# meta-pytorch/torchx

Hardware: AMD Instinct MI355X
Metric: tokens_per_second (higher is better)
Workload: dtype bf16; 1 GPU; model=llama3_8b, global_batch=4, seq_len=4096, parallelism=dp1

## Files before the change

torchx_amd/ops/csrc/attention.hip:

```cpp
#include "common.h"

#include <cstdlib>
#include <cstring>
#include <type_traits>

typedef __bf16 mbf16x8 __attribute__((ext_vector_type(8)));

#define HD 128
#define QBLK 32
#define KBLK 32
#define NWAVES 4
#define BLOCK_Q (QBLK * NWAVES)
#define BLOCK_K (KBLK * NWAVES)

__device__ __forceinline__ f32x16 mfma32(mbf16x8 a, mbf16x8 b, f32x16 c) {
  return __builtin_amdgcn_mfma_f32_32x32x16_bf16(a, b, c, 0, 0, 0);
}

__device__ __forceinline__ unsigned int pack_bf16x2(float a, float b) {
  unsigned int r;
  asm("v_cvt_pk_bf16_f32 %0, %1, %2" : "=v"(r) : "v"(a), "v"(b));
  return r;
}

__device__ __forceinline__ int c_row(int r, int half) {
  return (r & 3) + 8 * (r >> 2) + 4 * half;
}

__device__ __forceinline__ void cvals_to_frags(const float* p, bool hi,
                                               mbf16x8* f0, mbf16x8* f1) {
  unsigned int w[2][4];
  #pragma unroll
  for (int s = 0; s < 2; ++s) {
    unsigned int a01 = pack_bf16x2(p[8 * s + 0], p[8 * s + 1]);
    unsigned int a23 = pack_bf16x2(p[8 * s + 2], p[8 * s + 3]);
    unsigned int a45 = pack_bf16x2(p[8 * s + 4], p[8 * s + 5]);
    unsigned int a67 = pack_bf16x2(p[8 * s + 6], p[8 * s + 7]);
    unsigned int x01 = __shfl_xor((int)a01, 32, 64);
    unsigned int x23 = __shfl_xor((int)a23, 32, 64);
    unsigned int x45 = __shfl_xor((int)a45, 32, 64);
    unsigned int x67 = __shfl_xor((int)a67, 32, 64);
    w[s][0] = hi ? x45 : a01;
    w[s][1] = hi ? x67 : a23;
    w[s][2] = hi ? a45 : x01;
    w[s][3] = hi ? a67 : x23;
  }
  uint4_v u0 = {w[0][0], w[0][1], w[0][2], w[0][3]};
  uint4_v u1 = {w[1][0], w[1][1], w[1][2], w[1][3]};
  *f0 = __builtin_bit_cast(mbf16x8, u0);
  *f1 = __builtin_bit_cast(mbf16x8, u1);
}


#define FKV 64
#define KIMG_BYTES (FKV * 256)
#define VIMG_BYTES (HD * FKV * 2)
#define LOG2E 1.44269504088896340736f
#define LN2 0.69314718055994530942f

__device__ __forceinline__ mbf16x8 kimg_frag(const char* kimg, int sub, int c) {
  const int lane = threadIdx.x & 63;
  const int row = sub * 32 + (lane & 31);
  const int byte = (c * 32 + ((lane >> 5) * 16)) ^ ((row & 15) << 4);
  return *(const mbf16x8*)(kimg + row * 256 + byte);
}

__device__ __forceinline__ int vrot(int d) {
  return ((d >> 1) ^ (d >> 4)) & 7;
}

__device__ __forceinline__ mbf16x8 vimg_frag(const char* vimg, int dt, int ks) {
  const int lane = threadIdx.x & 63;
  const int d = dt * 32 + (lane & 31);
  const int g = (ks * 2 + (lane >> 5) + vrot(d)) & 7;
  return *(const mbf16x8*)(vimg + d * 128 + g * 16);
}

typedef short short4_v __attribute__((ext_vector_type(4)));
typedef __attribute__((address_space(3))) short4_v* lds_s4p;

__device__ __forceinline__ mbf16x8 nat_tr_frag(const char* nat, int ks,
                                               int dt) {
  const int lane = threadIdx.x & 63;
  const int j = lane & 15;
  const int r_lo = ks * 16 + ((lane >> 5) * 8) + (j >> 2);
  const int r_hi = r_lo + 4;
  const int d0 = dt * 32 + ((lane >> 4) & 1) * 16 + 4 * (j & 3);
  const int g16 = (d0 >> 3) << 4;
  const int off = (d0 & 7) * 2;
  const int b_lo = r_lo * 256 + ((g16 ^ ((r_lo & 15) << 4)) | off);
  const int b_hi = r_hi * 256 + ((g16 ^ ((r_hi & 15) << 4)) | off);
  short4_v lo = __builtin_amdgcn_ds_read_tr16_b64_v4i16(
      (lds_s4p)(nat + b_lo));
  short4_v hi = __builtin_amdgcn_ds_read_tr16_b64_v4i16(
      (lds_s4p)(nat + b_hi));
  uint2_v ul = __builtin_bit_cast(uint2_v, lo);
  uint2_v uh = __builtin_bit_cast(uint2_v, hi);
  uint4_v u = {ul[0], ul[1], uh[0], uh[1]};
  return __builtin_bit_cast(mbf16x8, u);
}

template <int NW = 4, int TFKV = FKV>
__device__ __forceinline__ void stage_k_glds(
    const unsigned short* __restrict__ kb, long kv0, long stride_elems,
    int S, char* kimg) {
  const int wave = threadIdx.x / 64;
  const int lane = threadIdx.x & 63;
  #pragma unroll
  for (int j = 0; j < (TFKV / 4) / NW; ++j) {
    const int i = wave * ((TFKV / 4) / NW) + j;
    const int row = i * 4 + (lane >> 4);
    const int colbyte = ((lane & 15) * 16) ^ ((row & 15) << 4);
    long srow = kv0 + row;
    if (srow >= S) srow = S - 1;
    const char* src = (const char*)(kb + srow * stride_elems) + colbyte;
    __builtin_amdgcn_global_load_lds(
        (const __attribute__((address_space(1))) unsigned int*)src,
        (__attribute__((address_space(3))) unsigned int*)(kimg + i * 1024),
        16, 0, 0);
  }
}

__device__ __forceinline__ void load_v_regs(
    const unsigned short* __restrict__ vb, long kv0, long stride_elems,
    int S, ushort8 vr[4]) {
  const int tid = threadIdx.x;
  #pragma unroll
  for (int p = 0; p < 4; ++p) {
    const int c = tid + p * 256;
    const int r = c >> 4, g = c & 15;
    long srow = kv0 + r;
    if (srow >= S) srow = S - 1;
    vr[p] = *(const ushort8*)(vb + srow * stride_elems + g * 8);
  }
}

__device__ __forceinline__ void write_v_tr(const ushort8 vr[4], char* vimg) {
  const int tid = threadIdx.x;
  #pragma unroll
  for (int p = 0; p < 4; ++p) {
    const int c = tid + p * 256;
    const int r = c >> 4, g = c & 15;
    #pragma unroll
    for (int j = 0; j < 8; ++j) {
      const int d = 8 * g + j;
      const int gr = ((r >> 3) + vrot(d)) & 7;
      *(unsigned short*)(vimg + d * 128 + gr * 16 + (r & 7) * 2) = vr[p][j];
    }
  }
}


__device__ __forceinline__ void map_block_fwd(int B, int Hq, int Hkv,
                                              int nqt, int G,
                                              int* b, int* hq, int* qt) {
  int bid = blockIdx.x;
  if (((B * Hkv) & 7) == 0) {
    const int gsz = G * nqt;
    const int xcd = bid & 7, slot = bid >> 3;
    const int g = (slot / gsz) * 8 + xcd;
    *b = g / Hkv;
    const int r = slot % gsz;
    *hq = (g % Hkv) * G + r / nqt;
    *qt = r % nqt;
  } else {
    *b = bid / (Hq * nqt);
    bid -= *b * Hq * nqt;
    *hq = bid / nqt;
    *qt = bid % nqt;
  }
}

__device__ __forceinline__ bool map_block_fwd_balanced(int B, int Hq, int Hkv,
                                                       int nqt, int G,
                                                       int heavy, int* b,
                                                       int* hq, int* qt) {
  const int xcd = blockIdx.x & 7, slot = blockIdx.x >> 3;
  const int u = slot / G;
  const int nstream = B * Hkv;
  int g, t;
  if ((nstream & 7) == 0) {
    const int ns = nstream >> 3;
    g = (u % ns) * 8 + xcd;
    t = u / ns;
  } else {
    const int unit = u * 8 + xcd;
    if (unit >= nstream * nqt) return false;
    g = unit % nstream;
    t = unit / nstream;
  }
  *b = g / Hkv;
  *hq = (g % Hkv) * G + slot % G;
  *qt = heavy ? nqt - 1 - t : t;
  return true;
}

template <int NTHREADS>
__device__ __forceinline__ void lds_nat_to_tr(const char* nat, char* tr_img) {
  const int tid = threadIdx.x;
  #pragma unroll
  for (int p = 0; p < 1024 / NTHREADS; ++p) {
    const int c = tid + p * NTHREADS;
    const int r = c >> 4, g = c & 15;
    const ushort8 v = *(const ushort8*)(
        nat + r * 256 + ((g * 16) ^ ((r & 15) << 4)));
    #pragma unroll
    for (int j = 0; j < 8; ++j) {
      const int d = 8 * g + j;
      const int gr = ((r >> 3) + vrot(d)) & 7;
      *(unsigned short*)(tr_img + d * 128 + gr * 16 + (r & 7) * 2) = v[j];
    }
  }
}



template <int NW = 4>
__device__ __forceinline__ void lds_nat_to_tr_own(const char* nat,
                                                  char* tr_img) {
  const int wave = threadIdx.x / 64;
  const int lane = threadIdx.x & 63;
  #pragma unroll
  for (int pp = 0; pp < 16 / NW; ++pp) {
    const int c = wave * (64 * 16 / NW) + pp * 64 + lane;
    const int r = c >> 4, g = c & 15;
    const ushort8 v = *(const ushort8*)(
        nat + r * 256 + ((g * 16) ^ ((r & 15) << 4)));
    #pragma unroll
    for (int j = 0; j < 8; ++j) {
      const int d = 8 * g + j;
      const int gr = ((r >> 3) + vrot(d)) & 7;
      *(unsigned short*)(tr_img + d * 128 + gr * 16 + (r & 7) * 2) = v[j];
    }
  }
}

template <int NW>
__global__ void __launch_bounds__(NW * 64, 2)
attn_fwd_kernel(const unsigned short* __restrict__ q,
                const unsigned short* __restrict__ k,
                const unsigned short* __restrict__ v,
                unsigned short* __restrict__ o,
                float* __restrict__ lse,
                int B, int S, int Hq, int Hkv, float scale, int causal,
                long q_rs, long kv_rs,
                int map) {
  __shared__ __align__(16) char smem[4 * KIMG_BYTES];

  const int BQ = NW * QBLK;
  const int nqt = (S + BQ - 1) / BQ;
  const int G = Hq / Hkv;
  int b, hq, qt;
  if (map == 0) {
    map_block_fwd(B, Hq, Hkv, nqt, G, &b, &hq, &qt);
  } else if (!map_block_fwd_balanced(B, Hq, Hkv, nqt, G, map == 1, &b, &hq,
                                     &qt)) {
    return;
  }
  const int hkv = hq / G;

  const int wave = threadIdx.x / 64;
  const int lane = threadIdx.x & 63;
  const bool hi = lane >= 32;
  const int qr = lane & 31;

  const long q_seq_stride = q_rs;
  const long kv_seq_stride = kv_rs;
  const unsigned short* qb = q + (long)b * S * q_seq_stride + (long)hq * HD;
  const unsigned short* kb = k + (long)b * S * kv_seq_stride + (long)hkv * HD;
  const unsigned short* vb = v + (long)b * S * kv_seq_stride + (long)hkv * HD;

  const int q0_blk = qt * BQ;
  const int qw0 = q0_blk + wave * QBLK;
  const long q_row = qw0 + qr;
  const bool wave_active = qw0 < S;

  mbf16x8 qfrag[8];
  {
    const long row = (q_row < S) ? q_row : (S - 1);
    const unsigned short* qp = qb + row * q_seq_stride + (hi ? 8 : 0);
    #pragma unroll
    for (int c = 0; c < 8; ++c) {
      qfrag[c] = __builtin_bit_cast(mbf16x8, *(const ushort8*)(qp + c * 16));
    }
  }

  f32x16 acc_o[4] = {};
  float m_run = -3.0e38f, l_run = 0.f;
  const float sc2 = scale * LOG2E;

  const int kv_limit = causal ? min(S, q0_blk + BQ) : S;
  const int ntiles = (kv_limit + FKV - 1) / FKV;
  const int qw_max = min(qw0 + QBLK - 1, S - 1);

  char* k0 = smem;
  char* k1 = smem + KIMG_BYTES;
  char* vcur = smem + 2 * KIMG_BYTES;
  char* vnxt = smem + 3 * KIMG_BYTES;

  stage_k_glds<NW>(kb, 0, kv_seq_stride, S, k0);
  stage_k_glds<NW>(vb, 0, kv_seq_stride, S, vcur);
  asm volatile("s_waitcnt vmcnt(0)");
  __syncthreads();

  for (int t = 0; t < ntiles; ++t) {
    const int kv0 = t * FKV;
    const bool has_next = (t + 1) < ntiles;
    if (has_next) {
      stage_k_glds<NW>(kb, kv0 + FKV, kv_seq_stride, S, k1);
      stage_k_glds<NW>(vb, kv0 + FKV, kv_seq_stride, S, vnxt);
    }

    const bool needed = wave_active && (!causal || kv0 <= qw_max);
    if (needed) {
      f32x16 acc0 = {}, acc1 = {};
      __builtin_amdgcn_s_setprio(1);
      #pragma unroll
      for (int c = 0; c < 8; ++c) {
        acc0 = mfma32(kimg_frag(k0, 0, c), qfrag[c], acc0);
        acc1 = mfma32(kimg_frag(k0, 1, c), qfrag[c], acc1);
      }
      __builtin_amdgcn_s_setprio(0);

      float sv[32];
      #pragma unroll
      for (int r = 0; r < 16; ++r) {
        sv[r] = acc0[r] * sc2;
        sv[16 + r] = acc1[r] * sc2;
      }
      const bool mask_tile =
          (causal && kv0 + FKV - 1 > qw0) || (kv0 + FKV > S) || (q_row >= S);
      if (mask_tile) {
        #pragma unroll
        for (int r = 0; r < 32; ++r) {
          const long kg = kv0 + (r >> 4) * 32 + c_row(r & 15, hi);
          if (kg >= S || q_row >= S || (causal && kg > q_row)) {
            sv[r] = -3.0e38f;
          }
        }
      }

      float m_tile = sv[0];
      #pragma unroll
      for (int r = 1; r < 32; ++r) m_tile = fmaxf(m_tile, sv[r]);
      m_tile = fmaxf(m_tile, __shfl_xor(m_tile, 32, 64));
      const float THR2 = 11.54f;
      if (!__all(m_tile - m_run <= THR2)) {
        const float m_new = fmaxf(m_run, m_tile);
        const float alpha = __builtin_amdgcn_exp2f(m_run - m_new);
        l_run *= alpha;
        m_run = m_new;
        #pragma unroll
        for (int dt = 0; dt < 4; ++dt) {
          #pragma unroll
          for (int r = 0; r < 16; ++r) acc_o[dt][r] *= alpha;
        }
      }

      float row_sum = 0.f;
      #pragma unroll
      for (int r = 0; r < 32; ++r) {
        sv[r] = __builtin_amdgcn_exp2f(sv[r] - m_run);
        row_sum += sv[r];
      }
      row_sum += __shfl_xor(row_sum, 32, 64);
      l_run += row_sum;

      mbf16x8 pf[4];
      cvals_to_frags(sv, hi, &pf[0], &pf[1]);
      cvals_to_frags(sv + 16, hi, &pf[2], &pf[3]);

      __builtin_amdgcn_s_setprio(1);
      #pragma unroll
      for (int dt = 0; dt < 4; ++dt) {
        #pragma unroll
        for (int ks = 0; ks < 4; ++ks) {
          acc_o[dt] = mfma32(nat_tr_frag(vcur, ks, dt), pf[ks], acc_o[dt]);
        }
      }
      __builtin_amdgcn_s_setprio(0);
    }

    if (has_next) {
      asm volatile("s_waitcnt vmcnt(0)");
      __syncthreads();
      char* tk = k0; k0 = k1; k1 = tk;
      char* tv = vcur; vcur = vnxt; vnxt = tv;
    }
  }

  if (!wave_active || q_row >= S) return;

  const float inv_l = (l_run > 0.f) ? 1.0f / l_run : 0.f;
  unsigned short* ob =
      o + (((long)b * S + q_row) * Hq + hq) * HD;
  #pragma unroll
  for (int dt = 0; dt < 4; ++dt) {
    #pragma unroll
    for (int g = 0; g < 4; ++g) {
      bf16x4_raw w;
      #pragma unroll
      for (int j = 0; j < 4; ++j) {
        w[j] = (short)f32_to_bf16(acc_o[dt][4 * g + j] * inv_l);
      }
      *(bf16x4_raw*)(ob + dt * 32 + 8 * g + 4 * (hi ? 1 : 0)) = w;
    }
  }
  if (!hi) {
    lse[((long)b * Hq + hq) * S + q_row] = (m_run + __log2f(l_run)) * LN2;
  }
// ... 695 lines not shown
  const int nt = (S + TFKV - 1) / TFKV;
  const int nt_eff = nt - t0;
  const int total = G * nt_eff;

  const bool ds_on = is_dk && ds != nullptr;
  const int ds_nqt = (S + BLOCK_Q - 1) / BLOCK_Q;
  const long ds_plane = ds_qt_base(ds_nqt, ds_nqt, causal);
  const long ds_lane = (long)(kw0 / KBLK) * (4 * DS_IMG_BYTES) + kr * 64 +
                       (hi ? 16 : 0);

  auto head_q = [&](int gh) {
    return q + (long)b * S * q_seq_stride + (long)(hkv * G + gh) * HD;
  };
  auto head_do = [&](int gh) {
    return dout + (long)b * S * dout_rs + (long)(hkv * G + gh) * HD;
  };
  auto stage_lse = [&](int gh, int t, int buf) {
    const int hq_ = hkv * G + gh;
    const int q0_ = t * TFKV;
    if (threadIdx.x < TFKV) {
      const float* lse_b = lse + ((long)b * Hq + hq_) * S;
      const int qg = q0_ + threadIdx.x;
      lse_buf[buf][threadIdx.x] = (qg < S) ? lse_b[qg] * LOG2E : 0.f;
    } else if (threadIdx.x < 2 * TFKV) {
      const float* del_b = delta + ((long)b * Hq + hq_) * S;
      const int qg = q0_ + (threadIdx.x - TFKV);
      del_buf[buf][threadIdx.x - TFKV] = (qg < S) ? del_b[qg] : 0.f;
    }
  };

  stage_k_glds8<TFKV>(head_q(0), (long)t0 * TFKV, q_seq_stride, S, qn_c);
  stage_k_glds8<TFKV>(head_do(0), (long)t0 * TFKV, dout_rs, S, don_c);
  asm volatile("s_waitcnt vmcnt(0)");
  stage_lse(0, t0, 0);
  __syncthreads();

  const float* lse_cur = lse_buf[0];
  const float* del_cur = del_buf[0];
  int lse_nxt = 1;
  for (int idx = 0; idx < total; ++idx) {
    const int gh = idx / nt_eff;
    const int t = t0 + idx % nt_eff;
    const int q0 = t * TFKV;
    const int hq = hkv * G + gh;
    const bool has_next = (idx + 1) < total;
    const int ngh = (idx + 1) / nt_eff;
    const long nrow0 = (long)(t0 + (idx + 1) % nt_eff) * TFKV;
    if (has_next) {
      stage_k_glds8<TFKV>(head_q(ngh), nrow0, q_seq_stride, S, qn_n);
      stage_k_glds8<TFKV>(head_do(ngh), nrow0, dout_rs, S, don_n);
    }

    const bool needed =
        wave_active && (!causal || q0 + TFKV - 1 >= kw0);
    int n_ds = 0;
    if (needed) {
      char* ds_head = ds + ((long)b * Hq + hq) * ds_plane * (4 * DS_IMG_BYTES)
                      + ds_lane;
      #pragma clang loop unroll(disable)
      for (int sb = 0; sb < TFKV / 32; ++sb) {
        if (causal && q0 + 32 * sb + 32 <= kw0) continue;
        f32x16 acc_s = {}, acc_dp = {};
        #pragma unroll
        for (int c = 0; c < 8; ++c) {
          acc_s = mfma32(kimg_frag(qn_c, sb, c), kfrag[c], acc_s);
          if (is_dk) {
            acc_dp = mfma32(kimg_frag(don_c, sb, c), vfrag[c], acc_dp);
          }
        }

        const int qs0 = q0 + 32 * sb;
        const bool mask_tile = (causal && qs0 < kw0 + 32)
                               || (qs0 + 32 > S) || !krow_valid;
        float cv[16];
        #pragma unroll
        for (int r = 0; r < 16; ++r) {
          const int ql = 32 * sb + c_row(r, hi);
          float s2 = acc_s[r] * sc2;
          if (mask_tile) {
            const long qg = q0 + ql;
            if (qg >= S || !krow_valid || (causal && k_row > qg)) {
              s2 = -3.0e38f;
            }
          }
          const float pr =
              __builtin_amdgcn_exp2f(s2 - lse_cur[ql]);
          cv[r] = is_dk ? scale * pr * (acc_dp[r] - del_cur[ql]) : pr;
        }

        mbf16x8 f0, f1;
        cvals_to_frags(cv, hi, &f0, &f1);

        const char* acc_img = is_dk ? qn_c : don_c;
        #pragma unroll
        for (int dt = 0; dt < 4; ++dt) {
          acc[dt] =
              mfma32(f0, nat_tr_frag(acc_img, 2 * sb, dt), acc[dt]);
          acc[dt] =
              mfma32(f1, nat_tr_frag(acc_img, 2 * sb + 1, dt), acc[dt]);
          if (dt == 0) {
            __builtin_amdgcn_sched_barrier(0);
            if (ds_on && qs0 < S) {
              char* p = ds_head +
                        (ds_qt_base(qs0 / BLOCK_Q, ds_nqt, causal) * 4 +
                         ((qs0 / QBLK) & 3)) * DS_IMG_BYTES;
              *(uint4_v*)p = __builtin_bit_cast(uint4_v, f0);
              *(uint4_v*)(p + 32) = __builtin_bit_cast(uint4_v, f1);
              n_ds = 2;
            }
          }
        }
      }
    }

    if (has_next) {
      if (n_ds) {
        asm volatile("s_waitcnt vmcnt(2)" ::: "memory");
      } else {
        asm volatile("s_waitcnt vmcnt(0)" ::: "memory");
      }
      stage_lse(ngh, t0 + (idx + 1) % nt_eff, lse_nxt);
      __syncthreads();
      lse_cur = lse_buf[lse_nxt];
      del_cur = del_buf[lse_nxt];
      lse_nxt ^= 1;
      char* tp;
      tp = qn_c; qn_c = qn_n; qn_n = tp;
      tp = don_c; don_c = don_n; don_n = tp;
    }
  }

  unsigned short* out = is_dk ? dk : dv;
  __syncthreads();
  float* tr = (float*)smem + wave * (32 * 36);
  if (wave_active) {
    #pragma unroll
    for (int dt = 0; dt < 4; ++dt) {
      __syncthreads();
      #pragma unroll
      for (int r = 0; r < 16; ++r) {
        tr[c_row(r, hi) * 36 + kr] = acc[dt][r];
      }
      __syncthreads();
      #pragma unroll
      for (int rep = 0; rep < 4; ++rep) {
        const int kk = kr;
        const int d0 = (hi ? 16 : 0) + rep * 4;
        if (kw0 + kk < S) {
          bf16x4_raw w;
          #pragma unroll
          for (int j = 0; j < 4; ++j) {
            w[j] = (short)f32_to_bf16(tr[kk * 36 + d0 + j]);
          }
          *(bf16x4_raw*)(out + ((long)b * S + kw0 + kk) * out_rs +
                         (long)hkv * HD + dt * 32 + d0) = w;
        }
      }
    }
  } else {
    #pragma unroll
    for (int i = 0; i < 8; ++i) __syncthreads();
  }
}

__device__ __forceinline__ void packed_to_frags_swap(const unsigned int* a,
                                                     mbf16x8* f0,
                                                     mbf16x8* f1) {
  unsigned int w[2][4];
  #pragma unroll
  for (int s = 0; s < 2; ++s) {
    auto e0 = __builtin_amdgcn_permlane32_swap(a[4 * s + 0], a[4 * s + 2],
                                               false, false);
    auto e1 = __builtin_amdgcn_permlane32_swap(a[4 * s + 1], a[4 * s + 3],
                                               false, false);
    w[s][0] = e0[0];
    w[s][1] = e1[0];
    w[s][2] = e0[1];
    w[s][3] = e1[1];
  }
  uint4_v u0 = {w[0][0], w[0][1], w[0][2], w[0][3]};
  uint4_v u1 = {w[1][0], w[1][1], w[1][2], w[1][3]};
  *f0 = __builtin_bit_cast(mbf16x8, u0);
  *f1 = __builtin_bit_cast(mbf16x8, u1);
}

template <int TFKV>
__global__ void __launch_bounds__(256, 1)
attn_bwd_dkv_merged_kernel(const unsigned short* __restrict__ q,
                           const unsigned short* __restrict__ k,
                           const unsigned short* __restrict__ v,
                           const unsigned short* __restrict__ dout,
                           const float* __restrict__ lse,
                           const float* __restrict__ delta,
                           unsigned short* __restrict__ dk,
                           unsigned short* __restrict__ dv,
                           char* __restrict__ ds,
                           int B, int S, int Hq, int Hkv, float scale,
                           int causal, long q_rs, long kv_rs, long dout_rs,
                           long out_rs) {
  constexpr int NS = TFKV / 32;
  __shared__ __align__(16) char smem[4 * (TFKV * 256)];
  __shared__ __align__(16) float lse_buf[2][TFKV], del_buf[2][TFKV];
  char* qn_c = smem;
  char* don_c = smem + TFKV * 256;
  char* qn_n = smem + 2 * (TFKV * 256);
  char* don_n = smem + 3 * (TFKV * 256);

  const int nkt = (S + BLOCK_K - 1) / BLOCK_K;
  const int G = Hq / Hkv;
  int b, hkv, kt;
  {
    int bid = blockIdx.x;
    if (((B * Hkv) & 7) == 0) {
      const int xcd = bid & 7, slot = bid >> 3;
      const int g = (slot / nkt) * 8 + xcd;
      b = g / Hkv;
      hkv = g % Hkv;
      kt = slot % nkt;
    } else {
      b = bid / (Hkv * nkt);
      bid -= b * Hkv * nkt;
      hkv = bid / nkt;
      kt = bid % nkt;
    }
  }

  const int wave = __builtin_amdgcn_readfirstlane(threadIdx.x / 64);
  const int lane = threadIdx.x & 63;
  const bool hi = lane >= 32;
  const int kr = lane & 31;

  const long q_seq_stride = q_rs;
  const long kv_seq_stride = kv_rs;
  const unsigned short* kb = k + (long)b * S * kv_seq_stride + (long)hkv * HD;
  const unsigned short* vb = v + (long)b * S * kv_seq_stride + (long)hkv * HD;

  const int kv0_blk = kt * BLOCK_K;
  const int kw0 = kv0_blk + wave * KBLK;
  const long k_row = kw0 + kr;
  const bool wave_active = kw0 < S;
  const bool krow_valid = k_row < S;

  mbf16x8 kfrag[8], vfrag[8];
  {
    const long row = krow_valid ? k_row : (S - 1);
    const unsigned short* kp = kb + row * kv_seq_stride + (hi ? 8 : 0);
    const unsigned short* vp = vb + row * kv_seq_stride + (hi ? 8 : 0);
    #pragma unroll
    for (int c = 0; c < 8; ++c) {
      kfrag[c] = __builtin_bit_cast(mbf16x8, *(const ushort8*)(kp + c * 16));
      vfrag[c] = __builtin_bit_cast(mbf16x8, *(const ushort8*)(vp + c * 16));
    }
  }

  f32x16 accv[4] = {}, acck[4] = {};
  const float sc2 = scale * LOG2E;

  const int t0 = causal ? (kv0_blk / TFKV) : 0;
  const int nt = (S + TFKV - 1) / TFKV;
  const int nt_eff = nt - t0;
  const int total = G * nt_eff;

  const bool ds_on = ds != nullptr;
  const int ds_nqt = (S + BLOCK_Q - 1) / BLOCK_Q;
  const long ds_plane = ds_qt_base(ds_nqt, ds_nqt, causal);
  const long ds_lane = (long)(kw0 / KBLK) * (4 * DS_IMG_BYTES) + kr * 64 +
                       (hi ? 16 : 0);

  auto head_q = [&](int gh) {
    return q + (long)b * S * q_seq_stride + (long)(hkv * G + gh) * HD;
  };
  auto head_do = [&](int gh) {
    return dout + (long)b * S * dout_rs + (long)(hkv * G + gh) * HD;
  };
  auto load_lse = [&](int gh, int t) -> float {
    const int hq_ = hkv * G + gh;
    const int q0_ = t * TFKV;
    float x = 0.f;
    if (threadIdx.x < TFKV) {
      const float* lse_b = lse + ((long)b * Hq + hq_) * S;
      const int qg = q0_ + threadIdx.x;
      x = (qg < S) ? lse_b[qg] : 0.f;
    } else if (threadIdx.x < 2 * TFKV) {
      const float* del_b = delta + ((long)b * Hq + hq_) * S;
      const int qg = q0_ + (threadIdx.x - TFKV);
      x = (qg < S) ? del_b[qg] : 0.f;
    }
    return x;
  };
  auto store_lse = [&](int buf, float x) {
    if (threadIdx.x < TFKV) {
      lse_buf[buf][threadIdx.x] = x * LOG2E;
    } else if (threadIdx.x < 2 * TFKV) {
      del_buf[buf][threadIdx.x - TFKV] = x;
    }
  };

  stage_k_glds<4, TFKV>(head_q(0), (long)t0 * TFKV, q_seq_stride, S, qn_c);
  stage_k_glds<4, TFKV>(head_do(0), (long)t0 * TFKV, dout_rs, S, don_c);
  asm volatile("s_waitcnt vmcnt(0)");
  store_lse(0, load_lse(0, t0));
  __syncthreads();

  const float* lse_cur = lse_buf[0];
  const float* del_cur = del_buf[0];
  int lse_nxt = 1;
  for (int idx = 0; idx < total; ++idx) {
    const int gh = idx / nt_eff;
    const int t = t0 + idx % nt_eff;
    const int q0 = t * TFKV;
    const int hq = hkv * G + gh;
    const bool has_next = (idx + 1) < total;
    const int ngh = (idx + 1) / nt_eff;
    const int ntile = t0 + (idx + 1) % nt_eff;
    float lse_reg = 0.f;
    if (has_next) {
      stage_k_glds<4, TFKV>(head_q(ngh), (long)ntile * TFKV, q_seq_stride, S,
                            qn_n);
      stage_k_glds<4, TFKV>(head_do(ngh), (long)ntile * TFKV, dout_rs, S,
                            don_n);
      lse_reg = load_lse(ngh, ntile);
    }

    int sb0 = 0;
    if (causal && kw0 > q0) sb0 = (kw0 - q0) / 32;
    if (!wave_active || sb0 > NS) sb0 = NS;
    sb0 = __builtin_amdgcn_readfirstlane(sb0);

    int n_ds = 0;
    char* ds_head = ds + ((long)b * Hq + hq) * ds_plane * (4 * DS_IMG_BYTES)
                    + ds_lane;

    auto load_frags = [&](int sb, mbf16x8* qf, mbf16x8* of) {
      #pragma unroll
      for (int c = 0; c < 8; ++c) {
        qf[c] = kimg_frag(qn_c, sb, c);
        of[c] = kimg_frag(don_c, sb, c);
      }
    };
    auto s_chain = [&](const mbf16x8* qf, const mbf16x8* of, f32x16& s_out,
                       f32x16& dp_out) {
      f32x16 s = {}, dp = {};
      #pragma unroll
      for (int c = 0; c < 8; ++c) {
        s = mfma32(qf[c], kfrag[c], s);
        dp = mfma32(of[c], vfrag[c], dp);
      }
      s_out = s;
      dp_out = dp;
    };

    if (sb0 < NS) {
      #pragma clang loop unroll(disable)
      for (int sbase = 0; sbase < NS; sbase += 2) {
        f32x16 acc_s[2], acc_dp[2];
        mbf16x8 qf[8], of[8];
        load_frags(sbase, qf, of);
        __builtin_amdgcn_sched_barrier(0);
        s_chain(qf, of, acc_s[0], acc_dp[0]);
        #pragma unroll
        for (int u = 0; u < 2; ++u) {
          const int sb = sbase + u;
          const bool nx = u == 0;
          const f32x16& cs = acc_s[u];
          const f32x16& cdp = acc_dp[u];
          if (nx) {
            #pragma unroll
            for (int c = 0; c < 4; ++c) {
              qf[c] = kimg_frag(qn_c, sb + 1, c);
              of[c] = kimg_frag(don_c, sb + 1, c);
            }
          }
          f32x4 lv[4], dl[4];
          lv[0] = *(const f32x4*)(lse_cur + 32 * sb + (hi ? 4 : 0));
          dl[0] = *(const f32x4*)(del_cur + 32 * sb + (hi ? 4 : 0));
          __builtin_amdgcn_sched_barrier(0);

          const int qs0 = q0 + 32 * sb;
          const bool mask_tile = (causal && qs0 < kw0 + 32)
                                 || (qs0 + 32 > S) || !krow_valid;
          mbf16x8 p0, p1, d0, d1;
          mbf16x8 tv[8], tk[8];
          auto stage_b = [&](auto masked) {
            float cp[16], cd[16];
            unsigned int pp[8], pd[8];
            f32x16 ns = {}, ndp = {};
            #pragma unroll
            for (int r = 0; r < 16; ++r) {
              if (nx) {
                if (r & 1) {
                  ndp = mfma32(of[r >> 1], vfrag[r >> 1], ndp);
                } else {
                  ns = mfma32(qf[r >> 1], kfrag[r >> 1], ns);
                }
                if (r < 8 && !(r & 1)) {
                  qf[4 + (r >> 1)] = kimg_frag(qn_c, sb + 1, 4 + (r >> 1));
                  of[4 + (r >> 1)] = kimg_frag(don_c, sb + 1, 4 + (r >> 1));
                }
              }
              if (r < 12 && !(r & 3)) {
                const int j = (r >> 2) + 1;
                lv[j] = *(const f32x4*)(lse_cur + 32 * sb + 8 * j +
                                        (hi ? 4 : 0));
                dl[j] = *(const f32x4*)(del_cur + 32 * sb + 8 * j +
                                        (hi ? 4 : 0));
              }
              if (r >= 8) {
                const int i = r - 8, dt = i >> 2;
                if (i & 2) {
                  tk[2 * dt + (i & 1)] =
                      nat_tr_frag(qn_c, 2 * sb + (i & 1), dt);
                } else {
                  tv[2 * dt + (i & 1)] =
                      nat_tr_frag(don_c, 2 * sb + (i & 1), dt);
                }
              }
              {
                #pragma clang fp contract(off)
                const int ql = 32 * sb + c_row(r, hi);
                float s2 = cs[r] * sc2;
                if (decltype(masked)::value) {
                  const long qg = q0 + ql;
                  if (qg >= S || !krow_valid || (causal && k_row > qg)) {
                    s2 = -3.0e38f;
                  }
                }
                const float pr =
                    __builtin_amdgcn_exp2f(s2 - lv[r >> 2][r & 3]);
                cp[r] = pr;
                cd[r] = scale * pr * (cdp[r] - dl[r >> 2][r & 3]);
              }
              if (r & 1) {
                pp[r >> 1] = pack_bf16x2(cp[r - 1], cp[r]);
                pd[r >> 1] = pack_bf16x2(cd[r - 1], cd[r]);
              }
              __builtin_amdgcn_sched_barrier(0);
            }
            if (nx) {
              acc_s[1] = ns;
              acc_dp[1] = ndp;
            }
            packed_to_frags_swap(pp, &p0, &p1);
            packed_to_frags_swap(pd, &d0, &d1);
          };
          if (mask_tile) {
            stage_b(std::true_type{});
          } else {
            stage_b(std::false_type{});
          }
          __builtin_amdgcn_sched_barrier(0);

          accv[0] = mfma32(p0, tv[0], accv[0]);
          accv[0] = mfma32(p1, tv[1], accv[0]);
          acck[0] = mfma32(d0, tk[0], acck[0]);
          acck[0] = mfma32(d1, tk[1], acck[0]);
          __builtin_amdgcn_sched_barrier(0);
          #pragma unroll
          for (int dt = 2; dt < 4; ++dt) {
            tv[2 * dt] = nat_tr_frag(don_c, 2 * sb, dt);
            tv[2 * dt + 1] = nat_tr_frag(don_c, 2 * sb + 1, dt);
            tk[2 * dt] = nat_tr_frag(qn_c, 2 * sb, dt);
            tk[2 * dt + 1] = nat_tr_frag(qn_c, 2 * sb + 1, dt);
          }
          __builtin_amdgcn_sched_barrier(0);
          if (ds_on && sb >= sb0 && qs0 < S) {
            char* p = ds_head +
                      (ds_qt_base(qs0 / BLOCK_Q, ds_nqt, causal) * 4 +
                       ((qs0 / QBLK) & 3)) * DS_IMG_BYTES;
            *(uint4_v*)p = __builtin_bit_cast(uint4_v, d0);
            *(uint4_v*)(p + 32) = __builtin_bit_cast(uint4_v, d1);
            n_ds = 2;
          }
          __builtin_amdgcn_sched_barrier(0);
          #pragma unroll
          for (int dt = 1; dt < 4; ++dt) {
            accv[dt] = mfma32(p0, tv[2 * dt], accv[dt]);
            accv[dt] = mfma32(p1, tv[2 * dt + 1], accv[dt]);
            acck[dt] = mfma32(d0, tk[2 * dt], acck[dt]);
            acck[dt] = mfma32(d1, tk[2 * dt + 1], acck[dt]);
          }
        }
      }
    }

    if (has_next) {
      if (n_ds) {
        asm volatile("s_waitcnt vmcnt(2)" ::: "memory");
      } else {
        asm volatile("s_waitcnt vmcnt(0)" ::: "memory");
      }
      store_lse(lse_nxt, lse_reg);
      asm volatile("s_waitcnt lgkmcnt(0)\n\ts_barrier" ::: "memory");
      lse_cur = lse_buf[lse_nxt];
      del_cur = del_buf[lse_nxt];
      lse_nxt ^= 1;
      char* tp;
      tp = qn_c; qn_c = qn_n; qn_n = tp;
      tp = don_c; don_c = don_n; don_n = tp;
    }
  }

  __syncthreads();
  float* tr = (float*)smem + wave * (32 * 36);
  if (wave_active) {
    #pragma unroll
    for (int o = 0; o < 2; ++o) {
      unsigned short* out = o ? dk : dv;
      #pragma unroll
      for (int dt = 0; dt < 4; ++dt) {
        __syncthreads();
        #pragma unroll
        for (int r = 0; r < 16; ++r) {
          tr[c_row(r, hi) * 36 + kr] = o ? acck[dt][r] : accv[dt][r];
        }
        __syncthreads();
        #pragma unroll
        for (int rep = 0; rep < 4; ++rep) {
          const int kk = kr;
          const int d0 = (hi ? 16 : 0) + rep * 4;
          if (kw0 + kk < S) {
            bf16x4_raw w;
            #pragma unroll
            for (int j = 0; j < 4; ++j) {
              w[j] = (short)f32_to_bf16(tr[kk * 36 + d0 + j]);
            }
            *(bf16x4_raw*)(out + ((long)b * S + kw0 + kk) * out_rs +
                           (long)hkv * HD + dt * 32 + d0) = w;
          }
        }
      }
    }
  } else {
    #pragma unroll
    for (int i = 0; i < 16; ++i) __syncthreads();
  }
}

#define ATTN_FWD_MAP_DEFAULT 1
static int g_fwd_map = -1;

extern "C" int attn_fwd_map_get() {
  if (g_fwd_map < 0) {
    const char* e = getenv("TORCHX_AMD_FWD_MAP");
    g_fwd_map = !e ? ATTN_FWD_MAP_DEFAULT
              : strcmp(e, "legacy") == 0 ? 0
              : strcmp(e, "balanced") == 0 ? 1
              : strcmp(e, "adjacent") == 0 ? 2 : ATTN_FWD_MAP_DEFAULT;
  }
  return g_fwd_map;
}

extern "C" void attn_fwd_map_set(int map) {
  g_fwd_map = (map >= 0 && map <= 2) ? map : ATTN_FWD_MAP_DEFAULT;
}

extern "C" void attn_fwd_launch(const void* q, const void* k, const void* v,
                                void* o, void* lse, int B, int S, int Hq,
                                int Hkv, float scale, int causal,
                                long q_rs, long kv_rs, hipStream_t stream) {
  static int fwd8 = -1;
  if (fwd8 < 0) {
    const char* e = getenv("TORCHX_AMD_FWD_8WAVE");
    fwd8 = (e && atoi(e)) ? 1 : 0;
  }
  if (fwd8 == 1) {
    const int nqt = (S + 8 * QBLK - 1) / (8 * QBLK);
    hipLaunchKernelGGL((attn_fwd_kernel<8>), dim3(B * Hq * nqt), dim3(512),
                       0, stream, (const unsigned short*)q,
                       (const unsigned short*)k, (const unsigned short*)v,
                       (unsigned short*)o, (float*)lse, B, S, Hq, Hkv,
                       scale, causal, q_rs, kv_rs, 0);
  } else {
    const int nqt = (S + 4 * QBLK - 1) / (4 * QBLK);
    const int map = attn_fwd_map_get();
    long grid = (long)B * Hq * nqt;
    if (map != 0 && ((B * Hkv) & 7) != 0) {
      grid = ((long)B * Hkv * nqt + 7) / 8 * 8 * (Hq / Hkv);
    }
    hipLaunchKernelGGL((attn_fwd_kernel<4>), dim3((unsigned)grid), dim3(256),
                       0, stream, (const unsigned short*)q,
                       (const unsigned short*)k, (const unsigned short*)v,
                       (unsigned short*)o, (float*)lse, B, S, Hq, Hkv,
                       scale, causal, q_rs, kv_rs, map);
  }
}

extern "C" void paged_prefill_attn_launch(
    const void* q, const void* kpool, const void* vpool, void* o,
    const void* bt, const void* ctx, int B, int S, int Hq, int Hkv,
    int num_pages, int logP, int M, float scale, hipStream_t stream) {
  const int nqt = (S + 4 * QBLK - 1) / (4 * QBLK);
  hipLaunchKernelGGL(paged_prefill_attn_kernel, dim3(B * Hq * nqt), dim3(256),
                     0, stream, (const unsigned short*)q,
                     (const unsigned short*)kpool,
                     (const unsigned short*)vpool, (unsigned short*)o,
                     (const int*)bt, (const int*)ctx, B, S, Hq, Hkv,
                     num_pages, logP, M, scale);
}

extern "C" void paged_prefill_attn_ragged_launch(
    const void* q, const void* kpool, const void* vpool, void* o,
    const void* bt, const void* ctx, const void* tiles, int ntiles, int B,
    int T, int Hq, int Hkv, int num_pages, int logP, int M, float scale,
    hipStream_t stream) {
  const long units = (long)ntiles * Hkv;
  const long grid = (units + 7) / 8 * 8 * (Hq / Hkv);
  hipLaunchKernelGGL(paged_prefill_attn_ragged_kernel, dim3((unsigned)grid),
                     dim3(256), 0, stream, (const unsigned short*)q,
                     (const unsigned short*)kpool,
                     (const unsigned short*)vpool, (unsigned short*)o,
                     (const int*)bt, (const int*)ctx, (const int4*)tiles,
                     ntiles, B, T, Hq, Hkv, num_pages, logP, M, scale);
}

static int g_dkv_merged = -1;

extern "C" int attn_bwd_dkv_impl_get() {
  if (g_dkv_merged < 0) {
    const char* e = getenv("TORCHX_AMD_DKV_IMPL");
    g_dkv_merged = (e && strcmp(e, "split") == 0) ? 0 : 1;
  }
  return g_dkv_merged;
}

extern "C" void attn_bwd_dkv_impl_set(int merged) {
  g_dkv_merged = merged ? 1 : 0;
}

extern "C" void attn_bwd_launch(const void* q, const void* k, const void* v,
                                const void* o, const void* dout,
                                const void* lse, void* delta, void* dq,
                                void* dk, void* dv, void* ds, int B, int S,
                                int Hq, int Hkv, float scale, int causal,
                                long q_rs, long kv_rs, long dqkv_q_rs,
                                long dqkv_kv_rs, hipStream_t stream) {
  const long rows = (long)B * S * Hq;
  hipLaunchKernelGGL(attn_bwd_pre_kernel, dim3((int)((rows + 15) / 16)),
                     dim3(256), 0, stream, (const unsigned short*)dout,
                     (const unsigned short*)o, (float*)delta, rows, S, Hq);
  const int nkt = (S + BLOCK_K - 1) / BLOCK_K;
  const long dout_rs = (long)Hq * HD;
  static int dkv_fkv = -1;
  if (dkv_fkv < 0) {
    const char* e = getenv("TORCHX_AMD_DKV_FKV");
    dkv_fkv = (e && atoi(e) == 64) ? 64 : 128;
  }
  if (attn_bwd_dkv_impl_get() == 1) {
    if (dkv_fkv == 128 && S % 128 == 0) {
      hipLaunchKernelGGL((attn_bwd_dkv_merged_kernel<128>),
                         dim3(B * Hkv * nkt), dim3(256), 0, stream,
                         (const unsigned short*)q, (const unsigned short*)k,
                         (const unsigned short*)v,
                         (const unsigned short*)dout, (const float*)lse,
                         (const float*)delta, (unsigned short*)dk,
                         (unsigned short*)dv, (char*)ds, B, S, Hq, Hkv,
                         scale, causal, q_rs, kv_rs, dout_rs, dqkv_kv_rs);
    } else {
      hipLaunchKernelGGL((attn_bwd_dkv_merged_kernel<64>),
                         dim3(B * Hkv * nkt), dim3(256), 0, stream,
                         (const unsigned short*)q, (const unsigned short*)k,
                         (const unsigned short*)v,
                         (const unsigned short*)dout, (const float*)lse,
                         (const float*)delta, (unsigned short*)dk,
                         (unsigned short*)dv, (char*)ds, B, S, Hq, Hkv,
                         scale, causal, q_rs, kv_rs, dout_rs, dqkv_kv_rs);
    }
  } else if (dkv_fkv == 128 && S % 128 == 0) {
    hipLaunchKernelGGL((attn_bwd_dkv_kernel<128>), dim3(B * Hkv * nkt),
                       dim3(512), 0, stream, (const unsigned short*)q,
                       (const unsigned short*)k, (const unsigned short*)v,
                       (const unsigned short*)dout, (const float*)lse,
                       (const float*)delta, (unsigned short*)dk,
                       (unsigned short*)dv, (char*)ds, B, S, Hq, Hkv,
                       scale, causal, q_rs, kv_rs, dout_rs, dqkv_kv_rs);
  } else {
    hipLaunchKernelGGL((attn_bwd_dkv_kernel<64>), dim3(B * Hkv * nkt),
                       dim3(512), 0, stream, (const unsigned short*)q,
                       (const unsigned short*)k, (const unsigned short*)v,
                       (const unsigned short*)dout, (const float*)lse,
                       (const float*)delta, (unsigned short*)dk,
                       (unsigned short*)dv, (char*)ds, B, S, Hq, Hkv,
                       scale, causal, q_rs, kv_rs, dout_rs, dqkv_kv_rs);
  }
  const int nqt = (S + BLOCK_Q - 1) / BLOCK_Q;
  if (ds != nullptr) {
    static int heavy_first = -1;
    if (heavy_first < 0) {
      const char* e = getenv("TORCHX_AMD_DQ_HEAVY_FIRST");
      heavy_first = (e && atoi(e) == 0) ? 0 : 1;
    }
    hipLaunchKernelGGL(attn_bwd_dq_stream_kernel, dim3(B * Hq * nqt),
                       dim3(256), 0, stream, (const unsigned short*)k,
                       (const char*)ds, (unsigned short*)dq, B, S, Hq, Hkv,
                       causal, kv_rs, dqkv_q_rs, heavy_first);
    return;
  }
  static int dq_fkv = -1;
  if (dq_fkv < 0) {
    const char* e = getenv("TORCHX_AMD_DQ_FKV");
    dq_fkv = (e && atoi(e) == 128) ? 128 : 64;
  }
  if (dq_fkv == 128 && S % 128 == 0) {
    hipLaunchKernelGGL((attn_bwd_dq_kernel<128>), dim3(B * Hq * nqt),
                       dim3(256), 0, stream, (const unsigned short*)q,
                       (const unsigned short*)k, (const unsigned short*)v,
                       (const unsigned short*)dout, (const float*)lse,
                       (const float*)delta, (unsigned short*)dq, B, S, Hq,
                       Hkv, scale, causal, q_rs, kv_rs, dqkv_q_rs);
  } else {
    hipLaunchKernelGGL((attn_bwd_dq_kernel<64>), dim3(B * Hq * nqt),
                       dim3(256), 0, stream, (const unsigned short*)q,
                       (const unsigned short*)k, (const unsigned short*)v,
                       (const unsigned short*)dout, (const float*)lse,
                       (const float*)delta, (unsigned short*)dq, B, S, Hq,
                       Hkv, scale, causal, q_rs, kv_rs, dqkv_q_rs);
  }
}
```

Baseline: 22890 tokens/s.

## Software-pipeline attention backward dK/dV loop across query sub-blocks

Restructures the inner loop of the attention backward dK/dV kernel into a fully unrolled, software-pipelined sequence. The previous sub-block's dV/dK accumulation MFMAs are interleaved with the current sub-block's softmax-gradient math and the next sub-block's S/dP MFMAs. LDS addresses are precomputed once per tile with immediate offsets, and the accumulators are pinned to AGPRs through empty inline asm. The goal is to hide LDS-read and exp latency behind matrix work, at the cost of higher register pressure and larger code.

```diff
diff --git a/torchx_amd/ops/csrc/attention.hip b/torchx_amd/ops/csrc/attention.hip
--- a/torchx_amd/ops/csrc/attention.hip
+++ b/torchx_amd/ops/csrc/attention.hip
@@ -106,6 +106,25 @@
     int S, char* kimg) {
   const int wave = threadIdx.x / 64;
   const int lane = threadIdx.x & 63;
+  #pragma unroll
+  for (int j = 0; j < (TFKV / 4) / NW; ++j) {
+    const int i = wave * ((TFKV / 4) / NW) + j;
+    const int row = i * 4 + (lane >> 4);
+    const int colbyte = ((lane & 15) * 16) ^ ((row & 15) << 4);
+    long srow = kv0 + row;
+    if (srow >= S) srow = S - 1;
+    const char* src = (const char*)(kb + srow * stride_elems) + colbyte;
+    __builtin_amdgcn_global_load_lds(
+        (const __attribute__((address_space(1))) unsigned int*)src,
+        (__attribute__((address_space(3))) unsigned int*)(kimg + i * 1024),
+        16, 0, 0);
+  }
+}
+
+template <int NW = 4, int TFKV = FKV>
+__device__ __forceinline__ void stage_k_glds_at(
+    const unsigned short* __restrict__ kb, long kv0, long stride_elems,
+    int S, char* kimg, int wave, int lane) {
   #pragma unroll
   for (int j = 0; j < (TFKV / 4) / NW; ++j) {
     const int i = wave * ((TFKV / 4) / NW) + j;
@@ -1407,9 +1426,12 @@
   store_lse(0, load_lse(0, t0));
   __syncthreads();
 
-  const float* lse_cur = lse_buf[0];
-  const float* del_cur = del_buf[0];
   int lse_nxt = 1;
+  auto pin_acc = [&]() __attribute__((always_inline)) {
+    asm volatile("" : "+a"(accv[0]), "+a"(accv[1]), "+a"(accv[2]),
+                      "+a"(accv[3]), "+a"(acck[0]), "+a"(acck[1]),
+                      "+a"(acck[2]), "+a"(acck[3]));
+  };
   for (int idx = 0; idx < total; ++idx) {
     const int gh = idx / nt_eff;
     const int t = t0 + idx % nt_eff;
@@ -1419,11 +1441,14 @@
     const int ngh = (idx + 1) / nt_eff;
     const int ntile = t0 + (idx + 1) % nt_eff;
     float lse_reg = 0.f;
+    int lane_t = lane;
+    asm volatile("" : "+v"(lane_t));
+    pin_acc();
     if (has_next) {
-      stage_k_glds<4, TFKV>(head_q(ngh), (long)ntile * TFKV, q_seq_stride, S,
-                            qn_n);
-      stage_k_glds<4, TFKV>(head_do(ngh), (long)ntile * TFKV, dout_rs, S,
-                            don_n);
+      stage_k_glds_at<4, TFKV>(head_q(ngh), (long)ntile * TFKV, q_seq_stride,
+                               S, qn_n, wave, lane_t);
+      stage_k_glds_at<4, TFKV>(head_do(ngh), (long)ntile * TFKV, dout_rs, S,
+                               don_n, wave, lane_t);
       lse_reg = load_lse(ngh, ntile);
     }
 
@@ -1436,153 +1461,223 @@
     char* ds_head = ds + ((long)b * Hq + hq) * ds_plane * (4 * DS_IMG_BYTES)
                     + ds_lane;
 
-    auto load_frags = [&](int sb, mbf16x8* qf, mbf16x8* of) {
-      #pragma unroll
-      for (int c = 0; c < 8; ++c) {
-        qf[c] = kimg_frag(qn_c, sb, c);
-        of[c] = kimg_frag(don_c, sb, c);
-      }
+    const int hi_t = lane_t >> 5;
+    const int img_off = (int)(qn_c - smem);
+    constexpr int DO_OFF = TFKV * 256;
+    int a_kf[8], a_tr[4];
+    {
+      const int kb = (lane_t & 31) * 256 +
+                     ((hi_t * 16) ^ ((lane_t & 15) << 4));
+      #pragma unroll
+      for (int c = 0; c < 8; ++c) a_kf[c] = img_off + (kb ^ (c * 32));
+      const int j = lane_t & 15;
+      const int rl = hi_t * 8 + (j >> 2);
+      const int g16 = ((lane_t >> 4) & 1) * 32 + ((j & 3) >> 1) * 16;
+      const int tb = rl * 256 + ((g16 ^ (rl << 4)) | ((j & 1) * 8));
+      #pragma unroll
+      for (int dt = 0; dt < 4; ++dt) a_tr[dt] = img_off + (tb ^ (dt * 64));
+    }
+    const float* lse_l = &lse_buf[lse_nxt ^ 1][hi_t * 4];
+    const float* del_l = &del_buf[lse_nxt ^ 1][hi_t * 4];
+    auto kf_read = [&](int o, int sb, int c)
+        __attribute__((always_inline)) {
+      return *(const mbf16x8*)(smem + a_kf[c] +
+                               ((o ? 0 : DO_OFF) + sb * 8192));
     };
-    auto s_chain = [&](const mbf16x8* qf, const mbf16x8* of, f32x16& s_out,
-                       f32x16& dp_out) {
-      f32x16 s = {}, dp = {};
-      #pragma unroll
-      for (int c = 0; c < 8; ++c) {
-        s = mfma32(qf[c], kfrag[c], s);
-        dp = mfma32(of[c], vfrag[c], dp);
-      }
-      s_out = s;
-      dp_out = dp;
+    auto acc_frag = [&](int sb, int i) __attribute__((always_inline)) {
+      const int dt = i >> 2;
+      const int imm = ((i & 1) ? 0 : DO_OFF) +
+                      (2 * sb + ((i >> 1) & 1)) * 4096;
+      short4_v lo = __builtin_amdgcn_ds_read_tr16_b64_v4i16(
+          (lds_s4p)(smem + a_tr[dt] + imm));
+      short4_v hh = __builtin_amdgcn_ds_read_tr16_b64_v4i16(
+          (lds_s4p)(smem + a_tr[dt ^ 1] + (imm + 1024)));
+      uint2_v ul = __builtin_bit_cast(uint2_v, lo);
+      uint2_v uh = __builtin_bit_cast(uint2_v, hh);
+      uint4_v u = {ul[0], ul[1], uh[0], uh[1]};
+      return __builtin_bit_cast(mbf16x8, u);
     };
+    auto acc_mfma = [&](int i, const mbf16x8& f, const mbf16x8& p0,
+                        const mbf16x8& p1, const mbf16x8& d0,
+                        const mbf16x8& d1) {
+      const int dt = i >> 2;
+      if (i & 1) {
+        acck[dt] = mfma32((i & 2) ? d1 : d0, f, acck[dt]);
+      } else {
+        accv[dt] = mfma32((i & 2) ? p1 : p0, f, accv[dt]);
+      }
+    };
+    auto export_ds = [&](int sb, const mbf16x8& d0, const mbf16x8& d1) {
+      const int qs0 = q0 + 32 * sb;
+      if (ds_on && sb >= sb0 && qs0 < S) {
+        char* p = ds_head +
+                  (ds_qt_base(qs0 / BLOCK_Q, ds_nqt, causal) * 4 +
+                   ((qs0 / QBLK) & 3)) * DS_IMG_BYTES;
+        *(uint4_v*)p = __builtin_bit_cast(uint4_v, d0);
+        *(uint4_v*)(p + 32) = __builtin_bit_cast(uint4_v, d1);
+        n_ds = 2;
+      }
+    };
 
     if (sb0 < NS) {
-      #pragma clang loop unroll(disable)
-      for (int sbase = 0; sbase < NS; sbase += 2) {
-        f32x16 acc_s[2], acc_dp[2];
+      f32x16 ns, ndp;
+      mbf16x8 p0, p1, d0, d1;
+
+      auto step_body = [&](int sb, auto has_prev, auto has_next,
+                           auto masked)
+          __attribute__((always_inline)) {
+        constexpr bool HP = decltype(has_prev)::value;
+        constexpr bool HN = decltype(has_next)::value;
+        const f32x16 cs = ns, cdp = ndp;
         mbf16x8 qf[8], of[8];
-        load_frags(sbase, qf, of);
+        mbf16x8 tf[16];
+        f32x4 lv[4], dl[4];
+        if (HN) {
+          qf[0] = kf_read(1, sb + 1, 0);
+          of[0] = kf_read(0, sb + 1, 0);
+        }
+        lv[0] = *(const f32x4*)(lse_l + 32 * sb);
+        dl[0] = *(const f32x4*)(del_l + 32 * sb);
+        if (HP) {
+          tf[0] = acc_frag(sb - 1, 0);
+          tf[1] = acc_frag(sb - 1, 1);
+          export_ds(sb - 1, d0, d1);
+        }
         __builtin_amdgcn_sched_barrier(0);
-        s_chain(qf, of, acc_s[0], acc_dp[0]);
-        #pragma unroll
-        for (int u = 0; u < 2; ++u) {
-          const int sb = sbase + u;
-          const bool nx = u == 0;
-          const f32x16& cs = acc_s[u];
-          const f32x16& cdp = acc_dp[u];
-          if (nx) {
-            #pragma unroll
-            for (int c = 0; c < 4; ++c) {
-              qf[c] = kimg_frag(qn_c, sb + 1, c);
-              of[c] = kimg_frag(don_c, sb + 1, c);
+
+        auto pair_reads = [&](int r) __attribute__((always_inline)) {
+          const int n = r + 2;
+          if (n < 16) {
+            if (HN) {
+              qf[n >> 1] = kf_read(1, sb + 1, n >> 1);
+              of[n >> 1] = kf_read(0, sb + 1, n >> 1);
+            }
+            if (HP) {
+              tf[n] = acc_frag(sb - 1, n);
+              tf[n + 1] = acc_frag(sb - 1, n + 1);
+            }
+            if (!(n & 3)) {
+              lv[n >> 2] = *(const f32x4*)(lse_l + 32 * sb + 2 * n);
+              dl[n >> 2] = *(const f32x4*)(del_l + 32 * sb + 2 * n);
             }
           }
-          f32x4 lv[4], dl[4];
-          lv[0] = *(const f32x4*)(lse_cur + 32 * sb + (hi ? 4 : 0));
-          dl[0] = *(const f32x4*)(del_cur + 32 * sb + (hi ? 4 : 0));
-          __builtin_amdgcn_sched_barrier(0);
-
-          const int qs0 = q0 + 32 * sb;
-          const bool mask_tile = (causal && qs0 < kw0 + 32)
-                                 || (qs0 + 32 > S) || !krow_valid;
-          mbf16x8 p0, p1, d0, d1;
-          mbf16x8 tv[8], tk[8];
-          auto stage_b = [&](auto masked) {
-            float cp[16], cd[16];
-            unsigned int pp[8], pd[8];
-            f32x16 ns = {}, ndp = {};
-            #pragma unroll
-            for (int r = 0; r < 16; ++r) {
-              if (nx) {
-                if (r & 1) {
-                  ndp = mfma32(of[r >> 1], vfrag[r >> 1], ndp);
-                } else {
-                  ns = mfma32(qf[r >> 1], kfrag[r >> 1], ns);
-                }
-                if (r < 8 && !(r & 1)) {
-                  qf[4 + (r >> 1)] = kimg_frag(qn_c, sb + 1, 4 + (r >> 1));
-                  of[4 + (r >> 1)] = kimg_frag(don_c, sb + 1, 4 + (r >> 1));
-                }
-              }
-              if (r < 12 && !(r & 3)) {
-                const int j = (r >> 2) + 1;
-                lv[j] = *(const f32x4*)(lse_cur + 32 * sb + 8 * j +
-                                        (hi ? 4 : 0));
-                dl[j] = *(const f32x4*)(del_cur + 32 * sb + 8 * j +
-                                        (hi ? 4 : 0));
-              }
-              if (r >= 8) {
-                const int i = r - 8, dt = i >> 2;
-                if (i & 2) {
-                  tk[2 * dt + (i & 1)] =
-                      nat_tr_frag(qn_c, 2 * sb + (i & 1), dt);
-                } else {
-                  tv[2 * dt + (i & 1)] =
-                      nat_tr_frag(don_c, 2 * sb + (i & 1), dt);
-                }
-              }
-              {
-                #pragma clang fp contract(off)
-                const int ql = 32 * sb + c_row(r, hi);
-                float s2 = cs[r] * sc2;
-                if (decltype(masked)::value) {
-                  const long qg = q0 + ql;
-                  if (qg >= S || !krow_valid || (causal && k_row > qg)) {
-                    s2 = -3.0e38f;
-                  }
-                }
-                const float pr =
-                    __builtin_amdgcn_exp2f(s2 - lv[r >> 2][r & 3]);
-                cp[r] = pr;
-                cd[r] = scale * pr * (cdp[r] - dl[r >> 2][r & 3]);
-              }
-              if (r & 1) {
-                pp[r >> 1] = pack_bf16x2(cp[r - 1], cp[r]);
-                pd[r >> 1] = pack_bf16x2(cd[r - 1], cd[r]);
-              }
+        };
+        float cp[16], cd[16];
+        unsigned int pp[8], pd[8];
+        f32x16 s_n = {}, dp_n = {};
+        #pragma unroll
+        for (int r = 0; r < 16; ++r) {
+          if (HN) {
+            if (r & 1) {
+              dp_n = mfma32(of[r >> 1], vfrag[r >> 1], dp_n);
+            } else {
+              s_n = mfma32(qf[r >> 1], kfrag[r >> 1], s_n);
+              __builtin_amdgcn_sched_barrier(0);
+              pair_reads(r);
               __builtin_amdgcn_sched_barrier(0);
             }
-            if (nx) {
-              acc_s[1] = ns;
-              acc_dp[1] = ndp;
+          }
+          if (HP) {
+            acc_mfma(r, tf[r], p0, p1, d0, d1);
+            if (!HN && !(r & 1)) {
+              __builtin_amdgcn_sched_barrier(0);
+              pair_reads(r);
+              __builtin_amdgcn_sched_barrier(0);
             }
-            packed_to_frags_swap(pp, &p0, &p1);
-            packed_to_frags_swap(pd, &d0, &d1);
-          };
-          if (mask_tile) {
-            stage_b(std::true_type{});
-          } else {
-            stage_b(std::false_type{});
+          }
+          {
+            #pragma clang fp contract(off)
+            const int ql = 32 * sb + c_row(r, hi);
+            float s2 = cs[r] * sc2;
+            if (decltype(masked)::value) {
+              const long qg = q0 + ql;
+              if (qg >= S || !krow_valid || (causal && k_row > qg)) {
+                s2 = -3.0e38f;
+              }
+            }
+            const float pr =
+                __builtin_amdgcn_exp2f(s2 - lv[r >> 2][r & 3]);
+            cp[r] = pr;
+            cd[r] = scale * pr * (cdp[r] - dl[r >> 2][r & 3]);
+          }
+          if (r & 1) {
+            if (r >= 3) pp[(r >> 1) - 1] = pack_bf16x2(cp[r - 3], cp[r - 2]);
+            pd[r >> 1] = pack_bf16x2(cd[r - 1], cd[r]);
           }
           __builtin_amdgcn_sched_barrier(0);
-
-          accv[0] = mfma32(p0, tv[0], accv[0]);
-          accv[0] = mfma32(p1, tv[1], accv[0]);
-          acck[0] = mfma32(d0, tk[0], acck[0]);
-          acck[0] = mfma32(d1, tk[1], acck[0]);
+        }
+        if (HN) {
+          ns = s_n;
+          ndp = dp_n;
+        }
+        packed_to_frags_swap(pd, &d0, &d1);
+        __builtin_amdgcn_sched_barrier(0);
+        pp[7] = pack_bf16x2(cp[14], cp[15]);
+        packed_to_frags_swap(pp, &p0, &p1);
+        __builtin_amdgcn_sched_barrier(0);
+      };
+      auto step = [&](int sb, auto has_prev, auto has_next)
+          __attribute__((always_inline)) {
+        const int qs0 = q0 + 32 * sb;
+        const bool mask_tile = (causal && qs0 < kw0 + 32)
+                               || (qs0 + 32 > S) || (kw0 + KBLK > S);
+        pin_acc();
+        if (mask_tile) {
+          step_body(sb, has_prev, has_next, std::true_type{});
+        } else {
+          step_body(sb, has_prev, has_next, std::false_type{});
+        }
+      };
+
+      pin_acc();
+      {
+        mbf16x8 qf[8], of[8];
+        #pragma unroll
+        for (int c = 0; c < 2; ++c) {
+          qf[c] = kf_read(1, 0, c);
+          of[c] = kf_read(0, 0, c);
+        }
+        __builtin_amdgcn_sched_barrier(0);
+        f32x16 s = {}, dp = {};
+        #pragma unroll
+        for (int c = 0; c < 8; ++c) {
+          s = mfma32(qf[c], kfrag[c], s);
+          if (!(c & 1) && c + 2 < 8) {
+            __builtin_amdgcn_sched_barrier(0);
+            #pragma unroll
+            for (int n = c + 2; n < c + 4; ++n) {
+              qf[n] = kf_read(1, 0, n);
+              of[n] = kf_read(0, 0, n);
+            }
+            __builtin_amdgcn_sched_barrier(0);
+          }
+          dp = mfma32(of[c], vfrag[c], dp);
+        }
+        ns = s;
+        ndp = dp;
+        __builtin_amdgcn_sched_barrier(0);
+      }
+      pin_acc();
+      step(0, std::false_type{}, std::true_type{});
+      #pragma unroll
+      for (int sb = 1; sb < NS - 1; ++sb) {
+        step(sb, std::true_type{}, std::true_type{});
+      }
+      step(NS - 1, std::true_type{}, std::false_type{});
+      {
+        mbf16x8 tf[16];
+        #pragma unroll
+        for (int i = 0; i < 4; ++i) tf[i] = acc_frag(NS - 1, i);
+        export_ds(NS - 1, d0, d1);
+        __builtin_amdgcn_sched_barrier(0);
+        #pragma unroll
+        for (int i = 0; i < 16; ++i) {
+          acc_mfma(i, tf[i], p0, p1, d0, d1);
           __builtin_amdgcn_sched_barrier(0);
-          #pragma unroll
-          for (int dt = 2; dt < 4; ++dt) {
-            tv[2 * dt] = nat_tr_frag(don_c, 2 * sb, dt);
-            tv[2 * dt + 1] = nat_tr_frag(don_c, 2 * sb + 1, dt);
-            tk[2 * dt] = nat_tr_frag(qn_c, 2 * sb, dt);
-            tk[2 * dt + 1] = nat_tr_frag(qn_c, 2 * sb + 1, dt);
-          }
-          __builtin_amdgcn_sched_barrier(0);
-          if (ds_on && sb >= sb0 && qs0 < S) {
-            char* p = ds_head +
-                      (ds_qt_base(qs0 / BLOCK_Q, ds_nqt, causal) * 4 +
-                       ((qs0 / QBLK) & 3)) * DS_IMG_BYTES;
-            *(uint4_v*)p = __builtin_bit_cast(uint4_v, d0);
-            *(uint4_v*)(p + 32) = __builtin_bit_cast(uint4_v, d1);
-            n_ds = 2;
-          }
-          __builtin_amdgcn_sched_barrier(0);
-          #pragma unroll
-          for (int dt = 1; dt < 4; ++dt) {
-            accv[dt] = mfma32(p0, tv[2 * dt], accv[dt]);
-            accv[dt] = mfma32(p1, tv[2 * dt + 1], accv[dt]);
-            acck[dt] = mfma32(d0, tk[2 * dt], acck[dt]);
-            acck[dt] = mfma32(d1, tk[2 * dt + 1], acck[dt]);
+          if (!(i & 3) && i + 4 < 16) {
+            #pragma unroll
+            for (int n = i + 4; n < i + 8; ++n) tf[n] = acc_frag(NS - 1, n);
+            __builtin_amdgcn_sched_barrier(0);
           }
         }
       }
@@ -1596,8 +1691,6 @@
       }
       store_lse(lse_nxt, lse_reg);
       asm volatile("s_waitcnt lgkmcnt(0)\n\ts_barrier" ::: "memory");
-      lse_cur = lse_buf[lse_nxt];
-      del_cur = del_buf[lse_nxt];
       lse_nxt ^= 1;
       char* tp;
       tp = qn_c; qn_c = qn_n; qn_n = tp;
```

Measured after the change: 23250 tokens/s (median of 6 runs). 1.02x the previous value.
